# nverchev/PointCloudCounterfactual

Hardware: AMD Instinct MI355X
Metric: clouds/sec Chamfer+EMD fwd+bwd, N=2048 B=32 (higher is better)
Workload: dtype f32; 1 GPU; BASELINE configs[1]+[2]: N=2048 B=32 per GPU, nn_distance (Chamfer, mean) fwd+bwd + match_cost (approxmatch+matchcost) fwd+bwd through the autograd surface; inputs = "recon" clouds (reference permuted + N(0, 0.02^2): a trained autoencoder, SURVEY 8(d)); the 8(d) stress set (both clouds i.i.d. U[0,1]^3) is value_stress (--full); emd_mode=implicit, batch_per_gpu=32, n_points=2048, global_batch=32, parallelism=batch-sharded x1, no data-path collective, launcher=single process

## Files before the change

pointcloudcounterfactual_amd/csrc/am_pair.hip:

```cpp
#include "approxmatch.hpp"
#include "wave_ops.hpp"

#include <algorithm>

namespace {

using pcc::sq3;

constexpr int kPairRB = 8;
constexpr int kPairPad = 65;

struct PairArgs {
    int n, m, n4, m4;
    const float *soa1, *soa2;
    const float *lv;
    LevelConsts lc;
    float cut2[kLevels];
    float *cost_part;
    float *part1;
    float *part2;
    int col_blocks, row_tiles, bc;
};

template <int Q, bool GRAD>
__global__ __launch_bounds__(256) void am_pair_kernel(PairArgs a) {
    __shared__ float4 lds_l[kPairRT][3];
    __shared__ int lds_mask[kPairRT];
    __shared__ float stash[GRAD ? 4 * kPairRB * 3 * kPairPad : 4];
    __shared__ float lds_red[4];
    const int tid = threadIdx.x, lane = tid & 63;
    const int w = __builtin_amdgcn_readfirstlane(tid >> 6);
    const int cbn = a.col_blocks, rtn = a.row_tiles;
    const int item = (int)blockIdx.x / a.bc, smp = (int)blockIdx.x - item * a.bc;
    const int shift_k = item / cbn, cblk = item - shift_k * cbn;
    const int base_r = (int)(((long long)(2 * cblk + 1) * rtn) / (2 * cbn));
    const int shift = ((shift_k + 1) >> 1) * ((shift_k & 1) ? 1 : -1);
    const int rtile = ((base_r + shift) % rtn + rtn) % rtn;
    const int l0 = rtile * kPairRT;
    const int kb = cblk * 64 * Q;
    const int k0 = kb + lane * Q;
    const size_t nm4 = (size_t)a.n4 + a.m4;
    const float *lvb = a.lv + (size_t)smp * kLevels * nm4;
    const float *s1 = a.soa1 + (size_t)smp * 3 * a.n4;
    const float *s2 = a.soa2 + (size_t)smp * 3 * a.m4;
    const int lcnt = min(kPairRT, a.m - l0);

    float rowx = 0.f, rowy = 0.f, rowz = 0.f, rowr[kLevels];
#pragma unroll
    for (int i = 0; i < kLevels; i++) rowr[i] = 0.f;
    if (tid < lcnt) {
        const int l = l0 + tid;
        rowx = s2[l];
        rowy = s2[a.m4 + l];
        rowz = s2[2 * a.m4 + l];
#pragma unroll
        for (int i = 0; i < kLevels; i++) rowr[i] = lvb[(size_t)i * nm4 + a.n4 + l];
    }
    float x1[Q], y1[Q], z1[Q], rl[kLevels][Q];
    float blo[3] = {__builtin_inff(), __builtin_inff(), __builtin_inff()};
    float bhi[3] = {-__builtin_inff(), -__builtin_inff(), -__builtin_inff()};
#pragma unroll
    for (int q = 0; q < Q; q++) {
        const bool real = k0 + q < a.n;
        const int k = real ? k0 + q : a.n - 1;
        x1[q] = s1[k];
        y1[q] = s1[a.n4 + k];
        z1[q] = s1[2 * a.n4 + k];
#pragma unroll
        for (int i = 0; i < kLevels; i++) rl[i][q] = real ? lvb[(size_t)i * nm4 + k] : 0.f;
        blo[0] = fminf(blo[0], x1[q]); bhi[0] = fmaxf(bhi[0], x1[q]);
        blo[1] = fminf(blo[1], y1[q]); bhi[1] = fmaxf(bhi[1], y1[q]);
        blo[2] = fminf(blo[2], z1[q]); bhi[2] = fmaxf(bhi[2], z1[q]);
    }
#pragma unroll
    for (int c = 0; c < 3; c++) {
#pragma unroll
        for (int off = 1; off < 64; off <<= 1) {
            blo[c] = fminf(blo[c], __shfl_xor(blo[c], off, 64));
            bhi[c] = fmaxf(bhi[c], __shfl_xor(bhi[c], off, 64));
        }
    }
    if (tid < lcnt) {
        const float bx = fmaxf(fmaxf(blo[0] - rowx, rowx - bhi[0]), 0.f);
        const float by = fmaxf(fmaxf(blo[1] - rowy, rowy - bhi[1]), 0.f);
        const float bz = fmaxf(fmaxf(blo[2] - rowz, rowz - bhi[2]), 0.f);
        const float bd2 = bx * bx + by * by + bz * bz;
        int mask = 0;
#pragma unroll
        for (int i = 0; i < kLevels; i++) mask |= (rowr[i] != 0.f && !(bd2 > a.cut2[i])) ? (1 << i) : 0;
        lds_l[tid][0] = make_float4(rowx, rowy, rowz, rowr[0]);
        lds_l[tid][1] = make_float4(rowr[1], rowr[2], rowr[3], rowr[4]);
        lds_l[tid][2] = make_float4(rowr[5], rowr[6], rowr[7], rowr[8]);
        lds_mask[tid] = mask;
    }
    float g1[Q][3];
#pragma unroll
    for (int q = 0; q < Q; q++) g1[q][0] = g1[q][1] = g1[q][2] = 0.f;
    float csum = 0.f;
    float *my_stash = stash + (GRAD ? w * kPairRB * 3 * kPairPad : 0);
    __syncthreads();

    for (int base = 0; base < lcnt; base += 4 * kPairRB) {
#pragma unroll 1
        for (int s = 0; s < kPairRB; s++) {
            const int li = base + 4 * s + w;
            float rx = 0.f, ry = 0.f, rz = 0.f;
            const int mask = li < lcnt ? __builtin_amdgcn_readfirstlane(lds_mask[li]) : 0;
            if (mask) {
                const float4 A = lds_l[li][0], B = lds_l[li][1], Cc = lds_l[li][2];
                const float rr[kLevels] = {A.w, B.x, B.y, B.z, B.w, Cc.x, Cc.y, Cc.z, Cc.w};
                float ex[Q], ey[Q], ez[Q], d[Q], acc[Q];
#pragma unroll
                for (int q = 0; q < Q; q++) {
                    ex[q] = A.x - x1[q];
                    ey[q] = A.y - y1[q];
                    ez[q] = A.z - z1[q];
                    d[q] = sq3(ex[q], ey[q], ez[q]);
                    acc[q] = 0.f;
                }
#pragma unroll
                for (int i = 0; i < kLevels; i++) {
                    if (mask & (1 << i)) {
#pragma unroll
                        for (int q = 0; q < Q; q++)
                            acc[q] = __builtin_fmaf(fast_exp2(a.lc.c[i] * d[q]) * rl[i][q], rr[i], acc[q]);
                    }
                }
#pragma unroll
                for (int q = 0; q < Q; q++) {
                    if (GRAD) {
                        float dm;
                        asm("v_max_f32 %0, %1, %2" : "=v"(dm) : "v"(d[q]), "v"(1e-20f));
                        const float f = acc[q] * __builtin_amdgcn_rsqf(dm);
                        csum = __builtin_fmaf(f, d[q], csum);
                        g1[q][0] = __builtin_fmaf(-ex[q], f, g1[q][0]);
                        g1[q][1] = __builtin_fmaf(-ey[q], f, g1[q][1]);
                        g1[q][2] = __builtin_fmaf(-ez[q], f, g1[q][2]);
                        rx = __builtin_fmaf(ex[q], f, rx);
                        ry = __builtin_fmaf(ey[q], f, ry);
                        rz = __builtin_fmaf(ez[q], f, rz);
                    } else {
                        csum = __builtin_fmaf(acc[q], __builtin_amdgcn_sqrtf(d[q]), csum);
                    }
                }
            }
            if (GRAD) {
                my_stash[(s * 3 + 0) * kPairPad + lane] = rx;
                my_stash[(s * 3 + 1) * kPairPad + lane] = ry;
                my_stash[(s * 3 + 2) * kPairPad + lane] = rz;
            }
        }
        if (GRAD) {
            const int v = lane % 24, h = lane / 24;
            float t = 0.f;
            __builtin_amdgcn_wave_barrier();
            if (lane < 48) {
                const float *src = my_stash + v * kPairPad + h * 32;
#pragma unroll 8
                for (int i = 0; i < 32; i++) t += src[i];
            }
            __builtin_amdgcn_wave_barrier();
            const float hi = __shfl(t, lane + 24, 64);
            const int sl = v / 3, c = v - sl * 3;
            const int li = base + 4 * sl + w;
            if (lane < 24 && li < lcnt)
                a.part2[(((size_t)smp * cbn + cblk) * a.m4 + (l0 + li)) * 3 + c] = t + hi;
        }
    }
    csum = pcc::wave_sum_down(csum);
    if (lane == 0) lds_red[w] = csum;
    __syncthreads();
    if (tid == 0)
        a.cost_part[(size_t)smp * cbn * rtn + rtile * cbn + cblk] =
            ((lds_red[0] + lds_red[1]) + lds_red[2]) + lds_red[3];
    if (GRAD) {
        static_assert(Q * 3 * 64 <= 4 * kPairRB * 3 * kPairPad, "column merge reuses the stash");
        for (int src = 1; src < 4; src++) {
            __syncthreads();
            if (w == src) {
#pragma unroll
                for (int q = 0; q < Q; q++)
#pragma unroll
                    for (int c = 0; c < 3; c++) stash[(q * 3 + c) * 64 + lane] = g1[q][c];
            }
            __syncthreads();
            if (w == 0) {
#pragma unroll
                for (int q = 0; q < Q; q++)
#pragma unroll
                    for (int c = 0; c < 3; c++) g1[q][c] += stash[(q * 3 + c) * 64 + lane];
            }
        }
        if (w == 0) {
            float *dst = a.part1 + (((size_t)smp * rtn + rtile) * a.n4) * 3;
#pragma unroll
            for (int q = 0; q < Q; q++) {
                if (k0 + q < a.n) {
#pragma unroll
                    for (int c = 0; c < 3; c++) dst[(size_t)(k0 + q) * 3 + c] = g1[q][c];
                }
            }
        }
    }
}

struct FinishArgs {
    int parts[3], npts[2], pitch[2];
    const float *part[3];
    const int *perm[2];
    const float *scale;
    float *out[3];
    const float *ch_d1, *ch_d2;
    float *ch_loss;
    int ch_n, ch_m, ch_mean;
    const int *flags;
};
__global__ __launch_bounds__(256) void pair_finish_kernel(FinishArgs f) {
    __shared__ float red[256];
    const int which = blockIdx.z, smp = blockIdx.y, tid = threadIdx.x;
    if (which == 3) {
        if (blockIdx.x) return;
        __shared__ float red2[256];
        float s1 = 0.f, s2 = 0.f;
        auto strided_sum = [&](const float *d, int cnt) -> float {
            float acc = 0.f;
            for (int i0 = tid; i0 < cnt; i0 += 8 * 256) {
                float v[8];
#pragma unroll
                for (int u = 0; u < 8; u++) v[u] = d[min(i0 + u * 256, cnt - 1)];
#pragma unroll
                for (int u = 0; u < 8; u++)
                    if (i0 + u * 256 < cnt) acc += v[u];
            }
            return acc;
        };
        s1 = strided_sum(f.ch_d1 + (size_t)smp * f.ch_n, f.ch_n);
        s2 = strided_sum(f.ch_d2 + (size_t)smp * f.ch_m, f.ch_m);
        red[tid] = s1;
        red2[tid] = s2;
        __syncthreads();
        for (int off = 128; off > 0; off >>= 1) {
            if (tid < off) {
                red[tid] += red[tid + off];
                red2[tid] += red2[tid + off];
            }
            __syncthreads();
        }
        if (tid == 0) f.ch_loss[smp] = f.ch_mean ? red2[0] / (float)f.ch_m + red[0] / (float)f.ch_n : red[0] + red2[0];
        return;
    }
    const bool poisoned = f.flags && (f.flags[(size_t)smp * kLiveRow + kInfSlot] | f.flags[(size_t)smp * kLiveRow + kInfSlot + 1] |
                                      f.flags[(size_t)smp * kLiveRow + kErrSlot]);
    if (which == 2) {
        if (blockIdx.x) return;
        const int parts = f.parts[2];
        float s = 0.f;
        for (int i = tid; i < parts; i += 256) s += f.part[2][(size_t)smp * parts + i];
        red[tid] = s;
        __syncthreads();
        for (int off = 128; off > 0; off >>= 1) {
            if (tid < off) red[tid] += red[tid + off];
            __syncthreads();
        }
        if (tid == 0) f.out[2][smp] = poisoned ? __builtin_nanf("") : red[0];
        return;
    }
    if (!f.out[which]) return;
    const int npts = f.npts[which], pitch = f.pitch[which], parts = f.parts[which];
    const int i = blockIdx.x * 256 + tid;
    if (i >= npts * 3) return;
    const int s = i / 3, c = i - s * 3;
    const float *p = f.part[which] + (size_t)smp * parts * pitch * 3 + i;
    const int pt = f.perm[which][(size_t)smp * npts + s];
    const size_t stride = (size_t)pitch * 3;
    float acc = p[0];
    int t = 1;
    for (; t + 8 <= parts; t += 8) {
        float v[8];
#pragma unroll
        for (int u = 0; u < 8; u++) v[u] = p[(size_t)(t + u) * stride];
#pragma unroll
        for (int u = 0; u < 8; u++) acc += v[u];
    }
    {
        float v[7];
#pragma unroll
        for (int u = 0; u < 7; u++) v[u] = p[(size_t)min(t + u, parts - 1) * stride];
#pragma unroll
        for (int u = 0; u < 7; u++)
            if (t + u < parts) acc += v[u];
    }
    f.out[which][((size_t)smp * npts + pt) * 3 + c] = poisoned ? __builtin_nanf("") : f.scale ? acc * f.scale[smp] : acc;
}

template <int Q>
int launch_pair(const PairArgs &pa, dim3 grid, bool grad, hipStream_t st) {
// ... 51 lines not shown
```

pointcloudcounterfactual_amd/csrc/approxmatch.hip:

```cpp
#include "approxmatch.hpp"
#include "pcc_test_hooks.h"
#include "wave_ops.hpp"

#include <algorithm>
#include <functional>
#include <mutex>
#include <type_traits>

namespace {

using pcc::sq3;
using pcc::WsView;

enum Phase { PH_A = 0, PH_B = 1, PH_CA = 2, PH_C = 3 };

__device__ __forceinline__ float pass_a_ratio(float remL, float sum) { return remL / (1e-9f + sum); }
struct PassB {
    float ratio, remain;
};
__device__ __forceinline__ PassB pass_b(float remR, float sum) {
    const float sumr = sum * remR;
    const float consumption = __builtin_fminf(remR / (sumr + 1e-9f), 1.0f);
    return {consumption * remR, __builtin_fmaxf(0.0f, remR - sumr)};
}
__device__ __forceinline__ float pass_c_left(float remL, float ratioL, float sum) { return __builtin_fmaxf(0.0f, remL - ratioL * sum); }

struct PhaseArgs {
    int n_own, n_cand, tiles, batch;
    int own_n4, cand_n4, own_nb, cand_nb;
    const float *own_soa, *cand_soa;
    const float *cand_box;
    const float *own_box16;
    const float *w0, *w1;
    long long w0_stride, w1_stride;
    float w0c;
    float c0, c1;
    float cut2;
    float cut2_fine;
    int first;
    int level;
    float multiL, multiR;
    float *remain;
    float *remain_out;
    long long remain_stride;
    const float *ratio_in;
    float *ratio_out;
    long long ratio_stride;
    float *clist;
    int *clist_cnt;
    int cl_n4;
    const unsigned *mask_in;
    unsigned *mask_out;
    int mask_words;
    const int *live_in;
    int *live_out;
};

enum Var { V_PLAIN = 0, V_CULL = 1, V_COWN = 3, V_CLIST = 4 };

struct Sched {
    int n, m, n4, m4, nb1, nb2;
    const float *soa1, *soa2, *box1, *box2;
    float *rem, *lv;
    float multiL, multiR;
    float *clist;
    int *clist_cnt;
    int *live_cnt;
    unsigned *live_mask;
    int skip;
    LevelConsts lc;
};

inline int sched_phases() { return 2 * kLevels + 1; }

inline PhaseArgs build_phase(const Sched &sc, int p, int *mode_out, int *var_out) {
    const long long nm4 = (long long)sc.n4 + sc.m4;
    const long long rs = (long long)sc.n4 + 2LL * sc.m4;
    PhaseArgs a{};
    a.multiL = sc.multiL;
    a.multiR = sc.multiR;
    const bool set1_owns = (p == 0) || (p % 2 == 0);
    if (set1_owns) {
        a.n_own = sc.n; a.n_cand = sc.m; a.own_n4 = sc.n4; a.cand_n4 = sc.m4; a.own_nb = sc.nb1; a.cand_nb = sc.nb2;
        a.own_soa = sc.soa1; a.cand_soa = sc.soa2; a.cand_box = sc.box2;
        a.own_box16 = sc.box1;
    } else {
        a.n_own = sc.m; a.n_cand = sc.n; a.own_n4 = sc.m4; a.cand_n4 = sc.n4; a.own_nb = sc.nb2; a.cand_nb = sc.nb1;
        a.own_soa = sc.soa2; a.cand_soa = sc.soa1; a.cand_box = sc.box1;
        a.own_box16 = sc.box2;
    }
    int mode, var;
    if (p == 0) {
        mode = PH_A;
        var = sc.skip ? V_CULL : V_PLAIN;
        a.level = 0;
        a.w0 = nullptr; a.w0c = sc.multiR; a.c0 = sc.lc.c[0]; a.first = 1;
        a.cut2 = zero_cut2(sc.lc, 0);
        a.ratio_out = sc.lv; a.ratio_stride = kLevels * nm4;
    } else {
        const int i = (p - 1) / 2;
        float *ratioL = sc.lv + (size_t)i * nm4, *ratioR = ratioL + sc.n4;
        a.level = i;
        a.first = (i == 0);
        a.c0 = sc.lc.c[i];
        if (p % 2 == 1) {
            mode = PH_B;
            var = !sc.skip ? V_PLAIN : i <= 2 ? V_CULL : V_COWN;
            a.w0 = ratioL; a.w0_stride = kLevels * nm4;
            a.cut2 = zero_cut2(sc.lc, i);
            a.remain = sc.rem + sc.n4 + (i & 1) * sc.m4;
            a.remain_out = sc.rem + sc.n4 + ((i + 1) & 1) * sc.m4;
            a.remain_stride = rs;
            a.ratio_out = ratioR; a.ratio_stride = kLevels * nm4;
            if (var == V_COWN) { a.clist = sc.clist; a.clist_cnt = sc.clist_cnt; a.cl_n4 = sc.m4; }
            if (sc.live_mask) {
                const int words = mask_words(sc.m4);
                a.mask_words = words;
                if (i + 1 < kLevels && (var == V_COWN || i == 2)) a.mask_out = sc.live_mask + (size_t)(i + 1) * words;
                if (var == V_COWN) {
                    a.mask_in = sc.live_mask + (size_t)i * words;
                    a.remain = a.remain_out = sc.rem + sc.n4 + sc.m4;
                }
            }
            if (sc.live_cnt) {
                a.live_in = (var == V_COWN && i >= 1) ? sc.live_cnt + i : nullptr;
                a.live_out = i + 1 < kLevels ? sc.live_cnt + i + 1 : nullptr;
            }
        } else {
            mode = i + 1 < kLevels ? PH_CA : PH_C;
            var = !sc.skip ? V_PLAIN : i <= 2 ? V_CULL : V_CLIST;
            if (var == V_CLIST) { a.clist = sc.clist; a.clist_cnt = sc.clist_cnt; a.cl_n4 = sc.m4; }
            a.w0 = ratioR; a.w0_stride = kLevels * nm4;
            a.w1 = sc.rem + sc.n4 + ((i + 1) & 1) * sc.m4; a.w1_stride = rs;
            a.remain = sc.rem; a.remain_stride = rs;
            a.ratio_in = ratioL; a.ratio_stride = kLevels * nm4;
            const int lc_i = i + 1 < kLevels ? i + 1 : i;
            a.cut2 = zero_cut2(sc.lc, lc_i);
            a.cut2_fine = zero_cut2(sc.lc, i);
            if (i + 1 < kLevels) {
                a.c1 = sc.lc.c[i + 1];
                a.ratio_out = sc.lv + (size_t)(i + 1) * nm4;
            }
        }
    }
    *mode_out = mode;
    *var_out = var;
    return a;
}

template <int NW, int R, int S, int CH>
struct PhaseLds {
    static constexpr int kC = (3 + NW) * CH;
    static constexpr int kRed = NW * S * 64 * R;
    static constexpr int kOwn = 64 * R;
    static constexpr int kWave = S;
    static constexpr int floats = kC + kRed + kOwn + kWave + 4;
};

template <int MODE, int R, int S, int CH, int VAR, int G = 1>
__device__ __forceinline__ void am_phase_body(const PhaseArgs &a, int smp, int tile, float *smem) {
    constexpr int T = 64 * S;
    constexpr int TQ = 64 * R / G;
    constexpr int PQ = 64 * R;
    static_assert(G == 1 || (VAR == V_COWN && R == 1), "lane-split owners: owner-compacted launches only");
    constexpr int NW = (MODE == PH_CA) ? 2 : 1;
    constexpr bool W0_CONST = (MODE == PH_A);
    constexpr bool COWN = VAR == V_COWN, CLIST = VAR == V_CLIST;
    static_assert(VAR == V_PLAIN || COWN || CLIST, "the box-culled passes run on am_fine_kernel");
    static_assert(!(CLIST && W0_CONST), "pass A of the first level has constant weights");
    static_assert(TQ <= T, "one epilogue owner per thread");
    using L = PhaseLds<NW, R, S, CH>;
    float *lds_c = smem;
    float *red = smem + L::kC;
    int *own_idx = reinterpret_cast<int *>(red + L::kRed);
    int *wave_cnt = own_idx + L::kOwn;

    const int tid = threadIdx.x;
    const int lane = tid & 63;
    const int w = __builtin_amdgcn_readfirstlane(tid >> 6);
    const int sub = G > 1 ? lane / TQ : 0;
    const float *O = a.own_soa + (size_t)smp * 3 * a.own_n4;
    const float *C = a.cand_soa + (size_t)smp * 3 * a.cand_n4;
    const float *W0 = W0_CONST ? nullptr : a.w0 + (size_t)smp * a.w0_stride;
    const float *W1 = (NW == 2) ? a.w1 + (size_t)smp * a.w1_stride : nullptr;

    if (!COWN && tile * TQ >= a.n_own) return;
    static_assert(CH / 4 <= T, "one float4 group per thread and chunk");
    float4 st_x, st_y, st_z, st_0, st_1;
    auto stage_load = [&](const float *Cc, const float *W0c, const float *W1c, int pitch, int q0, int ngroups) {
        const int i = min(tid, max(ngroups - 1, 0));
        st_x = reinterpret_cast<const float4 *>(Cc + q0)[i];
        st_y = reinterpret_cast<const float4 *>(Cc + (size_t)pitch + q0)[i];
        st_z = reinterpret_cast<const float4 *>(Cc + (size_t)2 * pitch + q0)[i];
        st_0 = make_float4(a.w0c, a.w0c, a.w0c, a.w0c);
        st_1 = st_0;
        if (!W0_CONST) st_0 = *reinterpret_cast<const float4 *>(W0c + q0 + 4 * i);
        if (NW == 2) st_1 = *reinterpret_cast<const float4 *>(W1c + q0 + 4 * i);
    };
    if (COWN) stage_load(C, W0, W1, a.cand_n4, 0, (min(CH, a.n_cand) + 3) / 4);
    int n_valid = min(TQ, a.n_own - tile * TQ);
    if (COWN) {
        const int lo = tile * TQ, hi = lo + TQ;
        const unsigned *mk = a.mask_in + (size_t)smp * kLevels * a.mask_words;
        unsigned *mnext = (tile == 0 && a.mask_out) ? a.mask_out + (size_t)smp * kLevels * a.mask_words : nullptr;
        const int wpt = (a.mask_words + T - 1) / T;
        unsigned word = 0;
        int mine = 0;
        if (wpt == 1) {
            word = mk[min(tid, a.mask_words - 1)];
            word &= -(unsigned)(tid < a.mask_words);
            if (mnext && tid < a.mask_words) atomicAnd(&mnext[tid], word);
            mine = __popc(word);
        } else {
            for (int j = tid * wpt; j < min(tid * wpt + wpt, a.mask_words); j++) {
                const unsigned wj = mk[j];
                if (mnext) atomicAnd(&mnext[j], wj);
                mine += __popc(wj);
            }
        }
        int incl = mine;
#pragma unroll
        for (int off = 1; off < 64; off <<= 1) {
            const int v = __shfl_up(incl, off, 64);
            incl += lane >= off ? v : 0;
        }
        if (lane == 63) wave_cnt[w] = incl;
        __syncthreads();
        int before = 0, total = 0;
#pragma unroll
        for (int i = 0; i < S; i++) {
            const int c = __builtin_amdgcn_readfirstlane(wave_cnt[i]);
            before += i < w ? c : 0;
            total += c;
        }
        int pos = before + incl - mine - lo;
        auto deal = [&](unsigned bits, int first_owner) {
            while (bits) {
                const int bit = __builtin_ctz(bits);
                bits &= bits - 1;
                if ((unsigned)pos < (unsigned)TQ) own_idx[pos] = first_owner + bit;
                pos++;
            }
        };
        if (wpt == 1) {
            deal(word, tid * 32);
        } else {
            for (int j = tid * wpt; j < min(tid * wpt + wpt, a.mask_words); j++) deal(mk[j], j * 32);
        }
        if (a.clist_cnt && tile == 0 && tid == 0) a.clist_cnt[smp] = total;
        n_valid = min(TQ, total - lo);
        if (n_valid <= 0) return;
        (void)hi;
        __syncthreads();
    }
    int own_e = -1;
    if (tid < TQ && tid < n_valid) own_e = COWN ? own_idx[tid] : tile * TQ + tid;

    float ox[R], oy[R], oz[R], s0[R], s1[R];
    float t0x = 0.f, t1x = 0.f;
#pragma unroll
    for (int r = 0; r < R; r++) {
        const int e = G > 1 ? (lane & (TQ - 1)) : r * 64 + lane;
        int o = COWN ? own_idx[e < n_valid ? e : 0] : tile * TQ + e;
        o = o < a.n_own ? o : a.n_own - 1;
        ox[r] = O[o];
        oy[r] = O[a.own_n4 + o];
        oz[r] = O[2 * a.own_n4 + o];
// ... 726 lines not shown
}

template <int MODE>
int launch_phase(const PhaseArgs &a, int b, int var, hipStream_t st, const char *what) {
    if (var == V_CULL) return launch_fine<MODE>(a, b, st, what);
    if (var == V_COWN) {
        if (a.live_in && a.level >= 5) return launch_phase_rs<MODE, 1, 8, 4>(a, b, var, st, what);
        if (a.live_in && a.level >= 4) return launch_phase_rs<MODE, 1, 8, 2>(a, b, var, st, what);
        return launch_phase_rs<MODE, 1, 8>(a, b, var, st, what);
    }
    const long long owners = (long long)b * a.n_own;
    if (var == V_CLIST && owners < 4LL * 65536) return launch_phase_rs<MODE, 1, 8>(a, b, var, st, what);
    if (owners >= 4LL * 65536) return launch_phase_rs<MODE, 4, 8>(a, b, var, st, what);
    if (owners >= 32768) return launch_phase_rs<MODE, 2, 8>(a, b, var, st, what);
    return launch_phase_rs<MODE, 1, 8>(a, b, var, st, what);
}

size_t cost_parts(int n, int m) { return (size_t)pcc::ceil_div(n, kMatKT) * pcc::ceil_div(m, kMatLT); }

struct WsLayout : pcc::AmDims {
    int b;
    int col_blocks, row_tiles;
    bool grad;
    size_t total;
    WsLayout(int b_, int n_, int m_, int col_blocks_ = 0, int row_tiles_ = 0, bool grad_ = false)
        : AmDims(n_, m_), b(b_), col_blocks(col_blocks_), row_tiles(row_tiles_), grad(grad_) {
        WsView unused;
        total = carve(0, 0, unused);
    }
    WsView view(char *base, int s) const {
        WsView v;
        carve(reinterpret_cast<uintptr_t>(base), (size_t)s, v);
        return v;
    }

  private:
    size_t carve(uintptr_t base, size_t s, WsView &v) const {
        size_t o = 0;
        auto sec = [&](auto *&p, size_t per) {
            using T = std::remove_reference_t<decltype(*p)>;
            p = reinterpret_cast<T *>(base + o + s * per * sizeof(T));
            o = (o + (size_t)b * per * sizeof(T) + 15) & ~(size_t)15;
        };
        sec(v.soa1, 3 * (size_t)n4);
        sec(v.soa2, 3 * (size_t)m4);
        sec(v.rank1, n);
        sec(v.rank2, m);
        sec(v.perm1, n);
        sec(v.perm2, m);
        sec(v.box1, (size_t)nb1 * 8);
        sec(v.box2, (size_t)nb2 * 8);
        sec(v.rem, rem_floats());
        sec(v.lv, lv_floats());
        sec(v.lv_orig, kLevels * ((size_t)n + m));
        sec(v.cpart, cost_parts(n, m));
        sec(v.clist, 5 * (size_t)m4);
        sec(v.clist_cnt, 1);
        sec(v.live_cnt, kLiveRow);
        sec(v.live_mask, (size_t)kLevels * mask_words(m4));
        sec(v.aos1, n);
        sec(v.aos2, m);
        sec(v.pair_cost, (size_t)col_blocks * row_tiles);
        sec(v.part1, grad ? (size_t)row_tiles * n4 * 3 : 0);
        sec(v.part2, grad ? (size_t)col_blocks * m4 * 3 : 0);
        return o;
    }
};

constexpr int kMaxLanes = 2;
hipStream_t side_stream() {
    static std::mutex mu;
    static hipStream_t streams[64] = {};
    int dev = 0;
    if (hipGetDevice(&dev) != hipSuccess || dev < 0 || dev >= 64) return nullptr;
    std::lock_guard<std::mutex> lk(mu);
    if (!streams[dev]) {
        int least = 0, greatest = 0;
        if (hipDeviceGetStreamPriorityRange(&least, &greatest) != hipSuccess) {
            (void)hipGetLastError();
            least = greatest = 0;
        }
        if (hipStreamCreateWithPriority(&streams[dev], hipStreamNonBlocking, greatest) != hipSuccess) {
            (void)hipGetLastError();
            if (hipStreamCreateWithFlags(&streams[dev], hipStreamNonBlocking) != hipSuccess) {
                streams[dev] = nullptr;
                (void)hipGetLastError();
            }
        }
    }
    return streams[dev];
}

struct ForkJoin {
    hipStream_t main, side = nullptr;
    ForkJoin(hipStream_t m, bool fork) : main(m) {
        if (!fork) return;
        hipEvent_t ev;
        if (hipEventCreateWithFlags(&ev, hipEventDisableTiming) != hipSuccess) return;
        if (hipEventRecord(ev, main) == hipSuccess) {
            hipStream_t s = side_stream();
            if (s && hipStreamWaitEvent(s, ev, 0) == hipSuccess) side = s;
        }
        (void)hipEventDestroy(ev);
    }
    ~ForkJoin() {
        if (!side) return;
        hipEvent_t ev;
        if (hipEventCreateWithFlags(&ev, hipEventDisableTiming) != hipSuccess) {
            (void)hipStreamSynchronize(side);
            return;
        }
        (void)hipEventRecord(ev, side);
        (void)hipStreamWaitEvent(main, ev, 0);
        (void)hipEventDestroy(ev);
    }
};

static bool resident_enabled() {
    return pcc::tuning(PCC_TUNE_AM_NORESIDENT) == 0;
}
int launch_fine_resident(const Sched &sc, int bc, hipStream_t st) {
    if (!sc.skip || !sc.live_cnt || !sc.live_mask || !resident_enabled()) return -1;
    if (sc.n > kFpCH || sc.m > kFpCH || sc.n < 1 || sc.m < 1) return -1;
    const int tiles = pcc::ceil_div(std::max(sc.n, sc.m), 64);
    FinePersistArgs a{};
    a.n = sc.n; a.m = sc.m; a.n4 = sc.n4; a.m4 = sc.m4; a.nb1 = sc.nb1; a.nb2 = sc.nb2; a.tiles = tiles;
    a.soa1 = sc.soa1; a.soa2 = sc.soa2; a.box1 = sc.box1; a.box2 = sc.box2;
    a.rem = sc.rem; a.lv = sc.lv; a.multiL = sc.multiL; a.multiR = sc.multiR;
    for (int i = 0; i < 4; i++) {
        a.c[i] = sc.lc.c[i];
        a.cut2[i] = zero_cut2(sc.lc, i);
    }
    a.live_cnt = sc.live_cnt;
    a.live_mask = sc.live_mask;
    a.mask_words = mask_words(sc.m4);
    static const int per_cu = [] {
        int r = 0;
        const void *k = reinterpret_cast<const void *>(am_fine_persist_kernel);
        if (hipOccupancyMaxActiveBlocksPerMultiprocessor(&r, k, 64 * kFineS, 0) != hipSuccess) (void)hipGetLastError();
        return r;
    }();
    if (per_cu < 2 || (long long)bc * tiles > pcc::device_cus()) return -1;
    pcc::CoresidentGate gate(pcc::kFineResident, st);
    if (!gate.ok) return -1;
    a.host_err = gate.sticky;
    a.inject = gate.inject;
    {
        pcc::ProfScope prof("am_fine_persist_kernel", st);
        hipLaunchKernelGGL(am_fine_persist_kernel, dim3((unsigned)(bc * tiles)), dim3(64 * kFineS), 0, st, a);
    }
    return pcc::check_launch("approxmatch(resident fine levels)");
}

Sched lane_sched(const WsLayout &L, const WsView &v, const LevelConsts &lc) {
    Sched sc{};
    sc.n = L.n; sc.m = L.m; sc.n4 = L.n4; sc.m4 = L.m4; sc.nb1 = L.nb1; sc.nb2 = L.nb2;
    sc.soa1 = v.soa1; sc.soa2 = v.soa2; sc.box1 = v.box1; sc.box2 = v.box2; sc.rem = v.rem; sc.lv = v.lv;
    if (L.n >= L.m) { sc.multiL = 1; sc.multiR = (float)(L.n / L.m); }
    else { sc.multiL = (float)(L.m / L.n); sc.multiR = 1; }
    sc.skip = cull_enabled() ? 1 : 0;
    sc.lc = lc;
    sc.clist = v.clist; sc.clist_cnt = v.clist_cnt;
    if (sc.skip) { sc.live_cnt = v.live_cnt; sc.live_mask = v.live_mask; }
    return sc;
}

int run_levels(const WsLayout &L, char *base, const float *xyz1, const float *xyz2, const LevelConsts &lc, hipStream_t st,
               const std::function<int(int, int, hipStream_t)> &lane_tail = nullptr,
               const std::function<int(int, int, hipStream_t)> &after_sort = nullptr) {
    if (const unsigned fw = pcc::take_coresident_failure(pcc::kFineResident)) {
        char buf[320];
        std::snprintf(buf, sizeof buf, "approxmatch: an earlier call on this device did not complete (a sample barrier of the resident "
                      "fine-level launch timed out: barrier %u of sample %u saw %u arrivals; the implicit path reported NaN for those "
                      "samples); this call was not started", (fw >> 4) & 0xfu, fw >> 20, (fw >> 8) & 0xfffu);
        return pcc::invalid(buf);
    }
    const bool split_enabled = pcc::tuning(PCC_TUNE_AM_NOSPLIT) == 0;

    struct Lane {
        int s0, bc;
        hipStream_t st;
        WsView v;
        Sched sc;
    };
    Lane lanes[kMaxLanes];
    int nlanes = 1;
    bool fork = false;
    if (split_enabled && L.b >= 8 && (long long)L.b * std::max(L.n, L.m) >= 32768) {
        fork = !pcc::capturing(st);
    }
    ForkJoin fj(st, fork);
    if (fj.side) nlanes = 2;
    for (int l = 0; l < nlanes; l++) {
        Lane &ln = lanes[l];
        ln.s0 = (int)((long long)L.b * l / nlanes);
        ln.bc = (int)((long long)L.b * (l + 1) / nlanes) - ln.s0;
        ln.st = l == 0 ? st : fj.side;
        ln.v = L.view(base, ln.s0);
        ln.sc = lane_sched(L, ln.v, lc);
    }
    int rc = PCC_OK;
    auto enqueue_head = [&](int l) -> int {
        const Lane &ln = lanes[l];
        const size_t s0 = (size_t)ln.s0;
        int r = pcc::sort_clouds(L, ln.v, ln.bc, xyz1 + s0 * L.n * 3, xyz2 + s0 * L.m * 3, (bool)after_sort, ln.st);
        if (!r && after_sort && l % 2 == 0) r = after_sort(ln.s0, ln.bc, ln.st);
        return r;
    };
    auto enqueue_pass = [&](int l, int p) -> int {
        const Lane &ln = lanes[l];
        int mode, var;
        const PhaseArgs a = build_phase(ln.sc, p, &mode, &var);
        switch (mode) {
        case PH_A: return launch_phase<PH_A>(a, ln.bc, var, ln.st, "approxmatch(A)");
        case PH_B: return launch_phase<PH_B>(a, ln.bc, var, ln.st, "approxmatch(B)");
        case PH_CA: return launch_phase<PH_CA>(a, ln.bc, var, ln.st, "approxmatch(CA)");
        default: return launch_phase<PH_C>(a, ln.bc, var, ln.st, "approxmatch(C)");
        }
    };
    int first_pass[kMaxLanes] = {};
    {
        for (int l = 0; l < nlanes && !rc; l++) rc = enqueue_head(l);
        if (rc) return rc;
        {
            pcc::ProfScope seq0("am_phase_sequence", lanes[0].st, true);
            pcc::ProfScope seq1("am_phase_sequence", lanes[nlanes > 1 ? 1 : 0].st, true, nlanes >= 2);
            for (int l = 0; l < nlanes && !rc; l++) {
                const int r = launch_fine_resident(lanes[l].sc, lanes[l].bc, lanes[l].st);
                if (r > 0) rc = r;
                else if (r == 0) first_pass[l] = kFpPasses;
            }
            for (int p = 0; p < sched_phases() && !rc; p++)
                for (int l = 0; l < nlanes && !rc; l++)
                    if (p >= first_pass[l]) rc = enqueue_pass(l, p);
            if (rc) return rc;
        }
        if (after_sort)
            for (int l = 1; l < nlanes; l += 2)
                if (int rc2 = after_sort(lanes[l].s0, lanes[l].bc, lanes[l].st)) return rc2;
        if (lane_tail) {
            for (int l = 0; l < nlanes; l++)
                if (int rc2 = lane_tail(lanes[l].s0, lanes[l].bc, lanes[l].st)) return rc2;
        }
    }
    return PCC_OK;
}

int approxmatch_impl(int b, int n, int m, const float *xyz1, const float *xyz2, float *match, float *temp,
                     void *workspace, size_t workspace_bytes, float *cost_out, hipStream_t st) {
    const WsLayout L(b, n, m);
    if (workspace_bytes < L.total) return pcc::invalid("approxmatch: workspace too small");
    if (!aligned16(workspace)) return pcc::invalid("approxmatch: workspace must be 16-byte aligned");
    char *base = static_cast<char *>(workspace);
    const LevelConsts lc = make_levels();
    int rc = run_levels(L, base, xyz1, xyz2, lc, st);
    if (rc) return rc;
    const WsView v = L.view(base, 0);
    hipLaunchKernelGGL(am_unpermute_kernel, dim3(pcc::ceil_div(n + m, 256), b), dim3(256), 0, st, n, m, L.n4, L.m4, v.lv, v.rem,
                       v.rank1, v.rank2, v.live_cnt, v.lv_orig, temp);
    rc = pcc::check_launch("approxmatch(unpermute)");
    if (rc) return rc;
    const dim3 grid(pcc::ceil_div(n, kMatKT), pcc::ceil_div(m, kMatLT), b);
    const bool vec = (n % 4 == 0) && aligned16(match);
    if (cost_out) {
        {
            pcc::ProfScope prof("am_materialise_kernel<cost>", st);
            if (vec) hipLaunchKernelGGL((am_materialise_kernel<true, true>), grid, dim3(256), 0, st, n, m, xyz1, xyz2, v.lv_orig, lc, match, v.cpart);
            else hipLaunchKernelGGL((am_materialise_kernel<true, false>), grid, dim3(256), 0, st, n, m, xyz1, xyz2, v.lv_orig, lc, match, v.cpart);
        }
        rc = pcc::check_launch("approxmatch(materialise+cost)");
        if (rc) return rc;
        pcc::launch_reduce_rows(b, (int)cost_parts(n, m), v.cpart, cost_out, st);
        return pcc::check_launch("approxmatch(cost reduce)");
    }
    {
        pcc::ProfScope prof("am_materialise_kernel", st);
        if (vec) hipLaunchKernelGGL((am_materialise_kernel<false, true>), grid, dim3(256), 0, st, n, m, xyz1, xyz2, v.lv_orig, lc, match, nullptr);
        else hipLaunchKernelGGL((am_materialise_kernel<false, false>), grid, dim3(256), 0, st, n, m, xyz1, xyz2, v.lv_orig, lc, match, nullptr);
    }
    return pcc::check_launch("approxmatch(materialise)");
}

int match_cost_implicit_impl(int b, int n, int m, const float *xyz1, const float *xyz2, const float *grad_cost,
                             float *cost, float *grad1, float *grad2, hipStream_t st,
                             const pcc::ChamferOut *chamfer = nullptr) {
    const bool grad = grad1 && grad2;
    const int col_blocks = pcc::ceil_div(n, 64 * kPairQ), row_tiles = pcc::ceil_div(m, kPairRT);
    const WsLayout L(b, n, m, col_blocks, row_tiles, grad);
    pcc::WsBlock ws(st);
    if (int rc = ws.alloc(L.total, "workspace allocation failed")) return rc;
    char *base = static_cast<char *>(ws.p);
    const LevelConsts lc = make_levels();
    auto tail = [&](int s0, int bc, hipStream_t lst) -> int {
        return pcc::launch_pair_finish(L, L.view(base, s0), s0, bc, col_blocks, row_tiles, grad_cost, cost, grad1, grad2, chamfer, lst);
    };
    auto nn_after_sort = [&](int s0, int bc, hipStream_t lst) -> int {
        return pcc::launch_nn_sorted(L, L.view(base, s0), s0, bc, chamfer, lst);
    };
    if (chamfer) return run_levels(L, base, xyz1, xyz2, lc, st, tail, nn_after_sort);
    return run_levels(L, base, xyz1, xyz2, lc, st, tail);
}

int approxmatch_entry(int b, int n, int m, const float *xyz1, const float *xyz2, float *match, float *temp, bool with_cost,
                      float *cost, hipStream_t st) {
    pcc::clear_error();
    if (int rc = check_sizes(with_cost ? "approxmatch_cost" : "approxmatch", b, n, m)) return rc;
    const char *null_ptr = with_cost ? "approxmatch_cost: null pointer" : "approxmatch: null pointer";
    if (b == 0) return PCC_OK;
    if (with_cost && !cost) return pcc::invalid(null_ptr);
    if (n == 0 || m == 0)
        return with_cost ? zero_fill_empty(b, n, m, cost, nullptr, nullptr, st, "approxmatch_cost: memset failed") : PCC_OK;
    if (!xyz1 || !xyz2 || !match || !temp) return pcc::invalid(null_ptr);
    pcc::WsBlock ws(st);
    const size_t bytes = WsLayout(b, n, m).total;
    if (int rc = ws.alloc(bytes, "workspace allocation failed")) return rc;
    return approxmatch_impl(b, n, m, xyz1, xyz2, match, temp, ws.p, bytes, cost, st);
}

}

namespace pcc {
int match_cost_with_chamfer(int b, int n, int m, const float *xyz1, const float *xyz2, float *cost, float *grad1,
                            float *grad2, hipStream_t st, const ChamferOut &chamfer) {
    return match_cost_implicit_impl(b, n, m, xyz1, xyz2, nullptr, cost, grad1, grad2, st, &chamfer);
}

}

extern "C" {

size_t pcc_approxmatch_workspace_bytes(int b, int n, int m) {
    if (b <= 0 || n <= 0 || m <= 0) return 0;
    return WsLayout(b, n, m).total;
}

int pcc_approxmatch_ws(int b, int n, int m, const float *xyz1, const float *xyz2, float *match, float *temp,
                       void *workspace, size_t workspace_bytes, pcc_stream_t stream) {
    pcc::clear_error();
    if (int rc = check_sizes("approxmatch", b, n, m)) return rc;
    if (b == 0 || n == 0 || m == 0) return PCC_OK;
    if (!xyz1 || !xyz2 || !match || !temp || !workspace) return pcc::invalid("approxmatch: null pointer");
    return approxmatch_impl(b, n, m, xyz1, xyz2, match, temp, workspace, workspace_bytes, nullptr,
                            static_cast<hipStream_t>(stream));
}

int pcc_approxmatch(int b, int n, int m, const float *xyz1, const float *xyz2, float *match, float *temp,
                    pcc_stream_t stream) {
    return approxmatch_entry(b, n, m, xyz1, xyz2, match, temp, false, nullptr, static_cast<hipStream_t>(stream));
}

int pcc_approxmatch_cost(int b, int n, int m, const float *xyz1, const float *xyz2, float *match, float *temp,
                         float *cost, pcc_stream_t stream) {
    return approxmatch_entry(b, n, m, xyz1, xyz2, match, temp, true, cost, static_cast<hipStream_t>(stream));
}

int pcc_match_cost(int b, int n, int m, const float *xyz1, const float *xyz2, const float *grad_cost, float *cost,
                   float *grad1, float *grad2, pcc_stream_t stream) {
    pcc::clear_error();
    if (int rc = check_sizes("match_cost", b, n, m)) return rc;
    if (b == 0) return PCC_OK;
    if (!cost) return pcc::invalid("match_cost: null pointer");
    hipStream_t st = static_cast<hipStream_t>(stream);
    if (n == 0 || m == 0) return zero_fill_empty(b, n, m, cost, grad1, grad2, st, "match_cost: memset failed");
    if (!xyz1 || !xyz2) return pcc::invalid("match_cost: null pointer");
    if ((grad1 == nullptr) != (grad2 == nullptr)) return pcc::invalid("match_cost: grad1 and grad2 go together");
    return match_cost_implicit_impl(b, n, m, xyz1, xyz2, grad_cost, cost, grad1, grad2, st);
}

void approxmatch(int b, int n, int m, const float *xyz1, const float *xyz2, float *match, float *temp,
                 pcc_stream_t stream) {
    (void)pcc_approxmatch(b, n, m, xyz1, xyz2, match, temp, stream);
}

}
```

Baseline: 72840 clouds/s.

## Skip dead row groups in pair kernel, vectorize loads, drop final phase in implicit mode

The pair kernel now builds a per-wave ballot of live rows up front and iterates only over live rows via ctz, zeroing stash or part2 entries for dead rows instead of looping through every slot. Column coordinate and level loads become single float4 loads per array, and the mask comes from a readlane of the preloaded ballot value. In implicit mode (when a lane_tail is present) the approxmatch schedule drops the last phase and stops emitting the candidate list at the final level, on the basis that the tail consumes the results directly. This adds assumptions that columns are float4-aligned and that the skipped last phase is not needed downstream.

```diff
diff --git a/pointcloudcounterfactual_amd/csrc/am_pair.hip b/pointcloudcounterfactual_amd/csrc/am_pair.hip
--- a/pointcloudcounterfactual_amd/csrc/am_pair.hip
+++ b/pointcloudcounterfactual_amd/csrc/am_pair.hip
@@ -56,21 +56,35 @@
 #pragma unroll
         for (int i = 0; i < kLevels; i++) rowr[i] = lvb[(size_t)i * nm4 + a.n4 + l];
     }
+    static_assert(Q == 4, "a lane loads its columns as one float4 per array");
     float x1[Q], y1[Q], z1[Q], rl[kLevels][Q];
     float blo[3] = {__builtin_inff(), __builtin_inff(), __builtin_inff()};
     float bhi[3] = {-__builtin_inff(), -__builtin_inff(), -__builtin_inff()};
-#pragma unroll
-    for (int q = 0; q < Q; q++) {
-        const bool real = k0 + q < a.n;
-        const int k = real ? k0 + q : a.n - 1;
-        x1[q] = s1[k];
-        y1[q] = s1[a.n4 + k];
-        z1[q] = s1[2 * a.n4 + k];
-#pragma unroll
-        for (int i = 0; i < kLevels; i++) rl[i][q] = real ? lvb[(size_t)i * nm4 + k] : 0.f;
-        blo[0] = fminf(blo[0], x1[q]); bhi[0] = fmaxf(bhi[0], x1[q]);
-        blo[1] = fminf(blo[1], y1[q]); bhi[1] = fmaxf(bhi[1], y1[q]);
-        blo[2] = fminf(blo[2], z1[q]); bhi[2] = fmaxf(bhi[2], z1[q]);
+    {
+        const int kc = min(k0, a.n4 - 4);
+        const float4 cx = *reinterpret_cast<const float4 *>(s1 + kc);
+        const float4 cy = *reinterpret_cast<const float4 *>(s1 + a.n4 + kc);
+        const float4 cz = *reinterpret_cast<const float4 *>(s1 + 2 * (size_t)a.n4 + kc);
+        float4 cr[kLevels];
+#pragma unroll
+        for (int i = 0; i < kLevels; i++) cr[i] = *reinterpret_cast<const float4 *>(lvb + (size_t)i * nm4 + kc);
+        const float lx = s1[a.n - 1], ly = s1[a.n4 + a.n - 1], lz = s1[2 * (size_t)a.n4 + a.n - 1];
+        const float vx[Q] = {cx.x, cx.y, cx.z, cx.w}, vy[Q] = {cy.x, cy.y, cy.z, cy.w}, vz[Q] = {cz.x, cz.y, cz.z, cz.w};
+#pragma unroll
+        for (int q = 0; q < Q; q++) {
+            const bool real = k0 + q < a.n;
+            x1[q] = real ? vx[q] : lx;
+            y1[q] = real ? vy[q] : ly;
+            z1[q] = real ? vz[q] : lz;
+#pragma unroll
+            for (int i = 0; i < kLevels; i++) {
+                const float vr[Q] = {cr[i].x, cr[i].y, cr[i].z, cr[i].w};
+                rl[i][q] = real ? vr[q] : 0.f;
+            }
+            blo[0] = fminf(blo[0], x1[q]); bhi[0] = fmaxf(bhi[0], x1[q]);
+            blo[1] = fminf(blo[1], y1[q]); bhi[1] = fmaxf(bhi[1], y1[q]);
+            blo[2] = fminf(blo[2], z1[q]); bhi[2] = fmaxf(bhi[2], z1[q]);
+        }
     }
 #pragma unroll
     for (int c = 0; c < 3; c++) {
@@ -100,48 +114,66 @@
     float *my_stash = stash + (GRAD ? w * kPairRB * 3 * kPairPad : 0);
     __syncthreads();
 
-    for (int base = 0; base < lcnt; base += 4 * kPairRB) {
+    const int mrow = 4 * (lane & 31) + w;
+    const int wmask = (lane < 32 && mrow < lcnt) ? lds_mask[mrow] : 0;
+    const unsigned live = (unsigned)__ballot(wmask != 0);
+    for (int base = 0, j0 = 0; base < lcnt; base += 4 * kPairRB, j0 += kPairRB) {
+        unsigned grp = (live >> j0) & ((1u << kPairRB) - 1);
+        if (GRAD) {
+            if (!grp) {
+                const int sl = lane / 3, c = lane - sl * 3;
+                const int li = base + 4 * sl + w;
+                if (lane < 24 && li < lcnt)
+                    a.part2[(((size_t)smp * cbn + cblk) * a.m4 + (l0 + li)) * 3 + c] = 0.f;
+                continue;
+            }
+            for (unsigned dead = ~grp & ((1u << kPairRB) - 1); dead; dead &= dead - 1) {
+                const int s = __builtin_ctz(dead);
+                my_stash[(s * 3 + 0) * kPairPad + lane] = 0.f;
+                my_stash[(s * 3 + 1) * kPairPad + lane] = 0.f;
+                my_stash[(s * 3 + 2) * kPairPad + lane] = 0.f;
+            }
+        }
 #pragma unroll 1
-        for (int s = 0; s < kPairRB; s++) {
+        for (; grp; grp &= grp - 1) {
+            const int s = __builtin_ctz(grp);
             const int li = base + 4 * s + w;
+            const float4 A = lds_l[li][0], B = lds_l[li][1], Cc = lds_l[li][2];
+            const int mask = __builtin_amdgcn_readlane(wmask, j0 + s);
             float rx = 0.f, ry = 0.f, rz = 0.f;
-            const int mask = li < lcnt ? __builtin_amdgcn_readfirstlane(lds_mask[li]) : 0;
-            if (mask) {
-                const float4 A = lds_l[li][0], B = lds_l[li][1], Cc = lds_l[li][2];
-                const float rr[kLevels] = {A.w, B.x, B.y, B.z, B.w, Cc.x, Cc.y, Cc.z, Cc.w};
-                float ex[Q], ey[Q], ez[Q], d[Q], acc[Q];
-#pragma unroll
-                for (int q = 0; q < Q; q++) {
-                    ex[q] = A.x - x1[q];
-                    ey[q] = A.y - y1[q];
-                    ez[q] = A.z - z1[q];
-                    d[q] = sq3(ex[q], ey[q], ez[q]);
-                    acc[q] = 0.f;
+            const float rr[kLevels] = {A.w, B.x, B.y, B.z, B.w, Cc.x, Cc.y, Cc.z, Cc.w};
+            float ex[Q], ey[Q], ez[Q], d[Q], acc[Q];
+#pragma unroll
+            for (int q = 0; q < Q; q++) {
+                ex[q] = A.x - x1[q];
+                ey[q] = A.y - y1[q];
+                ez[q] = A.z - z1[q];
+                d[q] = sq3(ex[q], ey[q], ez[q]);
+                acc[q] = 0.f;
+            }
+#pragma unroll
+            for (int i = 0; i < kLevels; i++) {
+                if (mask & (1 << i)) {
+#pragma unroll
+                    for (int q = 0; q < Q; q++)
+                        acc[q] = __builtin_fmaf(fast_exp2(a.lc.c[i] * d[q]) * rl[i][q], rr[i], acc[q]);
                 }
-#pragma unroll
-                for (int i = 0; i < kLevels; i++) {
-                    if (mask & (1 << i)) {
-#pragma unroll
-                        for (int q = 0; q < Q; q++)
-                            acc[q] = __builtin_fmaf(fast_exp2(a.lc.c[i] * d[q]) * rl[i][q], rr[i], acc[q]);
-                    }
-                }
-#pragma unroll
-                for (int q = 0; q < Q; q++) {
-                    if (GRAD) {
-                        float dm;
-                        asm("v_max_f32 %0, %1, %2" : "=v"(dm) : "v"(d[q]), "v"(1e-20f));
-                        const float f = acc[q] * __builtin_amdgcn_rsqf(dm);
-                        csum = __builtin_fmaf(f, d[q], csum);
-                        g1[q][0] = __builtin_fmaf(-ex[q], f, g1[q][0]);
-                        g1[q][1] = __builtin_fmaf(-ey[q], f, g1[q][1]);
-                        g1[q][2] = __builtin_fmaf(-ez[q], f, g1[q][2]);
-                        rx = __builtin_fmaf(ex[q], f, rx);
-                        ry = __builtin_fmaf(ey[q], f, ry);
-                        rz = __builtin_fmaf(ez[q], f, rz);
-                    } else {
-                        csum = __builtin_fmaf(acc[q], __builtin_amdgcn_sqrtf(d[q]), csum);
-                    }
+            }
+#pragma unroll
+            for (int q = 0; q < Q; q++) {
+                if (GRAD) {
+                    float dm;
+                    asm("v_max_f32 %0, %1, %2" : "=v"(dm) : "v"(d[q]), "v"(1e-20f));
+                    const float f = acc[q] * __builtin_amdgcn_rsqf(dm);
+                    csum = __builtin_fmaf(f, d[q], csum);
+                    g1[q][0] = __builtin_fmaf(-ex[q], f, g1[q][0]);
+                    g1[q][1] = __builtin_fmaf(-ey[q], f, g1[q][1]);
+                    g1[q][2] = __builtin_fmaf(-ez[q], f, g1[q][2]);
+                    rx = __builtin_fmaf(ex[q], f, rx);
+                    ry = __builtin_fmaf(ey[q], f, ry);
+                    rz = __builtin_fmaf(ez[q], f, rz);
+                } else {
+                    csum = __builtin_fmaf(acc[q], __builtin_amdgcn_sqrtf(d[q]), csum);
                 }
             }
             if (GRAD) {
diff --git a/pointcloudcounterfactual_amd/csrc/approxmatch.hip b/pointcloudcounterfactual_amd/csrc/approxmatch.hip
--- a/pointcloudcounterfactual_amd/csrc/approxmatch.hip
+++ b/pointcloudcounterfactual_amd/csrc/approxmatch.hip
@@ -68,10 +68,12 @@
     int *live_cnt;
     unsigned *live_mask;
     int skip;
+    int implicit;
     LevelConsts lc;
 };
 
 inline int sched_phases() { return 2 * kLevels + 1; }
+inline int sched_phases(const Sched &sc) { return sc.implicit ? sched_phases() - 1 : sched_phases(); }
 
 inline PhaseArgs build_phase(const Sched &sc, int p, int *mode_out, int *var_out) {
     const long long nm4 = (long long)sc.n4 + sc.m4;
@@ -112,7 +114,7 @@
             a.remain_out = sc.rem + sc.n4 + ((i + 1) & 1) * sc.m4;
             a.remain_stride = rs;
             a.ratio_out = ratioR; a.ratio_stride = kLevels * nm4;
-            if (var == V_COWN) { a.clist = sc.clist; a.clist_cnt = sc.clist_cnt; a.cl_n4 = sc.m4; }
+            if (var == V_COWN && !(sc.implicit && i + 1 == kLevels)) { a.clist = sc.clist; a.clist_cnt = sc.clist_cnt; a.cl_n4 = sc.m4; }
             if (sc.live_mask) {
                 const int words = mask_words(sc.m4);
                 a.mask_words = words;
@@ -1145,8 +1147,9 @@
     return pcc::check_launch("approxmatch(resident fine levels)");
 }
 
-Sched lane_sched(const WsLayout &L, const WsView &v, const LevelConsts &lc) {
+Sched lane_sched(const WsLayout &L, const WsView &v, const LevelConsts &lc, bool implicit) {
     Sched sc{};
+    sc.implicit = implicit ? 1 : 0;
     sc.n = L.n; sc.m = L.m; sc.n4 = L.n4; sc.m4 = L.m4; sc.nb1 = L.nb1; sc.nb2 = L.nb2;
     sc.soa1 = v.soa1; sc.soa2 = v.soa2; sc.box1 = v.box1; sc.box2 = v.box2; sc.rem = v.rem; sc.lv = v.lv;
     if (L.n >= L.m) { sc.multiL = 1; sc.multiR = (float)(L.n / L.m); }
@@ -1190,7 +1193,7 @@
         ln.bc = (int)((long long)L.b * (l + 1) / nlanes) - ln.s0;
         ln.st = l == 0 ? st : fj.side;
         ln.v = L.view(base, ln.s0);
-        ln.sc = lane_sched(L, ln.v, lc);
+        ln.sc = lane_sched(L, ln.v, lc, (bool)lane_tail);
     }
     int rc = PCC_OK;
     auto enqueue_head = [&](int l) -> int {
@@ -1223,7 +1226,7 @@
                 if (r > 0) rc = r;
                 else if (r == 0) first_pass[l] = kFpPasses;
             }
-            for (int p = 0; p < sched_phases() && !rc; p++)
+            for (int p = 0; p < sched_phases(lanes[0].sc) && !rc; p++)
                 for (int l = 0; l < nlanes && !rc; l++)
                     if (p >= first_pass[l]) rc = enqueue_pass(l, p);
             if (rc) return rc;
```

After: 75210 clouds/s, median of 6. 3.2% higher.
